# SJLeo/GCC

Measured on AMD Instinct MI355X. Metric: training images/sec at 256x256 (pix2pix GCC), higher is better.
Workload: dtype bf16; 1 GPU; Pix2Pix cityscapes 256x256 GCC distill+darts iteration (optimize_parameters + optimizer_netD_arch), student ngf32 / masked PatchGAN ndf128, teacher ngf64 / ndf128, filter_cfgs=None (no pretrained checkpoint to prune); batch_per_gpu=16, global_batch=16, image=256x256, parallelism=dp1, dropout=on (counter RNG; the oracle / golden iterations run --no_dropout)

## Files before the change

### gcc_amd/csrc/conv_wgrad.hip

```cpp
#include <mutex>
#include <string.h>
#include "common.hpp"

namespace {

struct WgradParams {
    const bf16_t* x;
    const bf16_t* dy;
    float* out;
    int N, H, W, ldx, xoff, Cip, Ci;
    int Ho, Wo, ldy, yoff, Co;
    int KH, KW, stride, pad;
    int ncols;
    int M;
    int ksteps_per_split;
    int col_tiles, co_tiles;
    uint32_t x_bytes, dy_bytes;
    FastDiv dHW, dW, dCip, dKW;
    int batch;
    long x_bstride, dy_bstride;
    int direct;
    int accumulate;
    float* dw;
    int rowmode;
    int debug;
};

constexpr int TP = 64;
constexpr uint32_t OOB = 0x7FFFFFF0u;

template <bool BIG>
struct WCfg {
    static constexpr int WAVES = BIG ? 8 : 4;
    static constexpr int NT = WAVES * 64;
    static constexpr int TCOL = BIG ? 256 : 128;
    static constexpr int TCO = BIG ? 256 : 128;
    static constexpr int RS = TCOL * 2;
    static constexpr int TILE_BYTES = TP * RS;
    static constexpr int CPR = RS / 16;
    static constexpr int RPP = 64 / CPR;
    static constexpr int WCOL = BIG ? 128 : 64;
    static constexpr int FI = WCOL / 16;
    static constexpr int FJ = 4;
    static constexpr int CH = BIG ? 16 : 8;
    static constexpr int TBL_BYTES = 2 * CH * TP * 8;
    static constexpr int LDS_BYTES = 4 * TILE_BYTES + TBL_BYTES;
};

__device__ __forceinline__ int phys_col_bytes(int row, int col_bytes) {
    return ((((col_bytes >> 5) ^ (row & 7)) << 5) | (col_bytes & 31));
}

template <int RS>
__device__ __forceinline__ bf16x8 tr_frag(const char* tile, int ks, int colbase, int lane) {
    const int g = lane >> 4, i = lane & 15;
    const int r0 = ks * 32 + 4 * g + (i >> 2), r1 = r0 + 16;
    const int cb = (colbase + 4 * (i & 3)) * 2;
    s16x4 lo = __builtin_amdgcn_ds_read_tr16_b64_v4i16(LDS_PTR(s16x4, tile + r0 * RS + phys_col_bytes(r0, cb)));
    s16x4 hi = __builtin_amdgcn_ds_read_tr16_b64_v4i16(LDS_PTR(s16x4, tile + r1 * RS + phys_col_bytes(r1, cb)));
    s16x8 v = {lo[0], lo[1], lo[2], lo[3], hi[0], hi[1], hi[2], hi[3]};
    return __builtin_bit_cast(bf16x8, v);
}

template <bool BIG, bool TABLE>
__device__ __forceinline__ void wgrad_body(const WgradParams& p, const int tile, const int split, const int bidx, char* smem) {
    using C = WCfg<BIG>;
    constexpr int RS = C::RS, TILE_BYTES = C::TILE_BYTES, FI = C::FI, FJ = C::FJ;
    char* sX = smem;
    char* sY = smem + 2 * TILE_BYTES;

    const int tid = threadIdx.x, lane = tid & 63;
    const int wave = __builtin_amdgcn_readfirstlane(tid >> 6);
    const int wa = wave & 1, wb = wave >> 1;

    const int ct = tile % p.col_tiles;
    const int ot = tile / p.col_tiles;
    const int col0 = ct * C::TCOL, co0 = ot * C::TCO;
    const int k_begin = split * p.ksteps_per_split;
    int k_end = k_begin + p.ksteps_per_split;
    const int ksteps_total = (p.M + TP - 1) / TP;
    if (k_end > ksteps_total) k_end = ksteps_total;

    const i32x4 rs_x = make_rsrc(p.x + (size_t)bidx * p.x_bstride, p.x_bytes);
    const i32x4 rs_y = make_rsrc(p.dy + (size_t)bidx * p.dy_bstride, p.dy_bytes);
    const uint32_t lds0 = (uint32_t)(uintptr_t)LDS_PTR(char, smem);

    const int rsub = lane / C::CPR, pch = lane % C::CPR;
    int q_tap_dy[4], q_tap_dx[4], q_cx[4], q_coy[4];
    bool q_colok[4], q_cook[4];
    int cxl[4], cyl[4];
    uint32_t xbits[4];
#pragma unroll
    for (int i = 0; i < 4; i++) {
        const int r7 = (C::RPP * (4 * wave + i) + rsub) & 7;
        const int lch = (((pch >> 1) ^ r7) << 1) | (pch & 1);
        const int q = col0 + lch * 8;
        q_colok[i] = q < p.ncols;
        const int tap = fdiv(q, p.dCip);
        q_cx[i] = q - tap * p.Cip;
        const int kh = fdiv(tap, p.dKW);
        const int kw = tap - kh * p.KW;
        q_tap_dy[i] = kh - p.pad; q_tap_dx[i] = kw - p.pad;
        q_coy[i] = co0 + lch * 8;
        q_cook[i] = q_coy[i] < ((p.Co + 7) & ~7);
        cxl[i] = ((kh * p.W + kw) * p.ldx + q_cx[i]) * 2;
        cyl[i] = q_cook[i] ? ((C::RPP * (4 * wave + i) + rsub) * p.ldy + p.yoff + q_coy[i]) * 2 : (int)0x80000000u;
        xbits[i] = q_colok[i] ? (0x80000000u | (1u << (kh & 15)) | (1u << (16 + (kw & 15)))) : 0x80008000u;
    }

    char* tbl = smem + 4 * TILE_BYTES;
    const int nk = k_end - k_begin;
    auto build_chunk = [&](int c) {
        for (int e = tid; e < C::CH * TP; e += C::NT) {
            const int step = c * C::CH + (e >> 6);
            const int m = (k_begin + step) * TP + (e & 63);
            i32x2 ent = {0, 0};
            if (step < nk && m < p.M) {
                const int n = fdiv(m, p.dHW);
                const int r = m - n * (p.Ho * p.Wo);
                const int oy = fdiv(r, p.dW);
                const int ox = r - oy * p.Wo;
                const int iy0 = oy * p.stride - p.pad, ix0 = ox * p.stride - p.pad;
                uint32_t mask = 0x80000000u;
                for (int k = 0; k < p.KH; k++) mask |= ((unsigned)(iy0 + k) < (unsigned)p.H) ? (1u << k) : 0u;
                for (int k = 0; k < p.KW; k++) mask |= ((unsigned)(ix0 + k) < (unsigned)p.W) ? (1u << (16 + k)) : 0u;
                ent[0] = (((n * p.H + iy0) * p.W + ix0) * p.ldx + p.xoff) * 2;
                ent[1] = (int)mask;
            }
            *(i32x2*)(tbl + ((c & 1) * (C::CH * TP) + e) * 8) = ent;
        }
    };
    const int tl = (C::RPP * 4 * wave + rsub) * 8;
    auto issue_loads = [&](int kstep, int stage) {
        const char* te = tbl + (kstep & (2 * C::CH - 1)) * (TP * 8) + tl;
        const int sby = (k_begin + kstep) * TP * p.ldy * 2;
#pragma unroll
        for (int i = 0; i < 4; i++) {
            uint32_t offx, offy;
            if constexpr (!TABLE) {
                const int row = C::RPP * (4 * wave + i) + rsub;
                const int m = (k_begin + kstep) * TP + row;
                const bool mv = m < p.M;
                const int n = fdiv(m, p.dHW);
                const int r = m - n * (p.Ho * p.Wo);
                const int oy = fdiv(r, p.dW);
                const int ox = r - oy * p.Wo;
                const int iy = oy * p.stride + q_tap_dy[i], ix = ox * p.stride + q_tap_dx[i];
                const bool okx = mv && q_colok[i] && (unsigned)iy < (unsigned)p.H && (unsigned)ix < (unsigned)p.W;
                offx = okx ? (uint32_t)((((n * p.H + iy) * p.W + ix) * p.ldx + p.xoff + q_cx[i]) * 2) : OOB;
                const bool oky = mv && q_cook[i];
                offy = oky ? (uint32_t)((m * p.ldy + p.yoff + q_coy[i]) * 2) : OOB;
            } else {
                const i32x2 ent = *(const i32x2*)(te + i * (C::RPP * 8));
                const uint32_t mask = (uint32_t)ent[1];
// ... 269 lines not shown
    const int split = blockIdx.z;
    const int b_begin = split * p.blocks_per_split;
    int b_end = b_begin + p.blocks_per_split;
    if (b_end > p.blocks) b_end = p.blocks;
    const int nb = b_end - b_begin;

    const i32x4 rs_x = make_rsrc(p.x, p.x_bytes);
    const i32x4 rs_y = make_rsrc(p.dy, p.dy_bytes);
    const uint32_t lds0 = (uint32_t)(uintptr_t)LDS_PTR(char, smem);

    const int rsub = lane >> 3, pch = lane & 7;
    int yl[YJ], ypy[YJ], ypx[YJ];
#pragma unroll
    for (int j = 0; j < YJ; j++) {
        const int row = 8 * (wave + NW * j) + rsub;
        const int lch = (((pch >> 1) ^ ((row >> 1) & 3)) << 1) | (pch & 1);
        ypy[j] = row >> 4; ypx[j] = row & 15;
        yl[j] = ((ypy[j] * p.Wo + ypx[j]) * p.ldy + p.yoff + co0 + lch * 8) * 2;
    }
    int xl[XJ], xhy[XJ], xhx[XJ];
#pragma unroll
    for (int j = 0; j < XJ; j++) {
        const int row = 8 * (wave + NW * j) + rsub;
        const int lch = (((pch >> 1) ^ ((row >> 1) & 3)) << 1) | (pch & 1);
        xhy[j] = row / HP; xhx[j] = row - xhy[j] * HP;
        xl[j] = ((xhy[j] * p.W + xhx[j]) * p.ldx + p.xoff + ci0 + lch * 8) * 2;
        if (xhx[j] >= HW) xhx[j] = 1 << 20;
    }
    const int mine = ((C::YP - 1 - wave) / NW + 1) + ((C::XP - 1 - wave) / NW + 1);
    auto issue = [&](int b, int stage) {
        const int n = fdiv(b, p.dT);
        const int t = b - n * (p.TY * p.TX);
        const int ty = fdiv(t, p.dTX);
        const int Y0 = ty * TR, X0 = (t - ty * p.TX) * TW;
        const int ybase = ((n * p.Ho + Y0) * p.Wo + X0) * p.ldy * 2;
        const int xbase = ((n * p.H + Y0 - 1) * p.W + X0 - 1) * p.ldx * 2;
        const uint32_t d0 = lds0 + stage * STAGE;
#pragma unroll
        for (int j = 0; j < YJ; j++) {
            if ((j + 1) * NW <= C::YP || wave + NW * j < C::YP) {
                const bool ok = Y0 + ypy[j] < p.Ho && X0 + ypx[j] < p.Wo;
                lds_dma16(rs_y, d0 + (wave + NW * j) * 1024, ok ? (uint32_t)(ybase + yl[j]) : OOB);
            }
        }
#pragma unroll
        for (int j = 0; j < XJ; j++) {
            if ((j + 1) * NW <= C::XP || wave + NW * j < C::XP) {
                const bool ok = (unsigned)(Y0 - 1 + xhy[j]) < (unsigned)p.H && (unsigned)(X0 - 1 + xhx[j]) < (unsigned)p.W;
                lds_dma16(rs_x, d0 + Y_BYTES + (wave + NW * j) * 1024, ok ? (uint32_t)(xbase + xl[j]) : OOB);
            }
        }
    };

    const int g = lane >> 4, li = lane & 15;
    const int px = 4 * g + (li >> 2);
    const int kh = KS == 4 ? wave >> 1 : wave / 3, kw0 = KS == 4 ? 2 * (wave & 1) : wave - 3 * (wave / 3);
    int ya[4], xa[TPW][4];
#pragma unroll
    for (int t = 0; t < 4; t++) {
        ya[t] = px * RSB + ((t ^ ((px >> 1) & 3)) << 5) + 8 * (li & 3);
#pragma unroll
        for (int tj = 0; tj < TPW; tj++) {
            const int hrow = kh * HP + px + kw0 + tj;
            xa[tj][t] = Y_BYTES + hrow * RSB + ((t ^ ((hrow >> 1) & 3)) << 5) + 8 * (li & 3);
        }
    }

    f32x4 acc[TPW][4][4];
#pragma unroll
    for (int a = 0; a < TPW; a++)
#pragma unroll
        for (int i = 0; i < 4; i++)
#pragma unroll
            for (int j = 0; j < 4; j++) acc[a][i][j] = f32x4{0.f, 0.f, 0.f, 0.f};

    if (nb > 0) {
        issue(b_begin, 0);
        if (nb > 1) issue(b_begin + 1, 1);
        int cur = 0, fill = 2;
        for (int b = 0; b < nb; b++) {
            if (b + 1 < nb) {
                if (mine == 7) asm volatile("s_waitcnt vmcnt(7)" ::: "memory");
                else if (mine == 6) asm volatile("s_waitcnt vmcnt(6)" ::: "memory");
                else if (mine == 5) asm volatile("s_waitcnt vmcnt(5)" ::: "memory");
                else asm volatile("s_waitcnt vmcnt(4)" ::: "memory");
            } else {
                asm volatile("s_waitcnt vmcnt(0)" ::: "memory");
            }
            __syncthreads();
            if (b + 2 < nb) issue(b_begin + b + 2, fill);
            const char* st = smem + cur * STAGE;
#pragma unroll
            for (int pp = 0; pp < 2; pp++) {
                bf16x8 fx[2][TPW * 4], fy[2][4];
#pragma unroll
                for (int k2 = 0; k2 < 2; k2++) {
                    const int ks = 2 * pp + k2;
#pragma unroll
                    for (int tj = 0; tj < TPW; tj++)
#pragma unroll
                        for (int t = 0; t < 4; t++)
                            fx[k2][tj * 4 + t] = ts_frag(st + xa[tj][t] + 2 * ks * (HP * RSB), HP * RSB);
#pragma unroll
                    for (int t = 0; t < 4; t++) fy[k2][t] = ts_frag(st + ya[t] + 2 * ks * (TW * RSB), TW * RSB);
                }
#pragma unroll
                for (int k2 = 0; k2 < 2; k2++)
#pragma unroll
                    for (int i = 0; i < TPW * 4; i++)
#pragma unroll
                        for (int j = 0; j < 4; j++)
                            acc[i >> 2][i & 3][j] = __builtin_amdgcn_mfma_f32_16x16x32_bf16(fx[k2][i], fy[k2][j], acc[i >> 2][i & 3][j], 0, 0, 0);
                if constexpr (KS == 4) {
                    __builtin_amdgcn_sched_group_barrier(0x100, 24, 0);
#pragma unroll
                    for (int r = 0; r < 12; r++) {
                        __builtin_amdgcn_sched_group_barrier(0x008, 2, 0);
                        __builtin_amdgcn_sched_group_barrier(0x100, 2, 0);
                    }
                    __builtin_amdgcn_sched_group_barrier(0x008, 40, 0);
                } else {
                    __builtin_amdgcn_sched_group_barrier(0x100, 16, 0);
#pragma unroll
                    for (int r = 0; r < 8; r++) {
                        __builtin_amdgcn_sched_group_barrier(0x008, 2, 0);
                        __builtin_amdgcn_sched_group_barrier(0x100, 2, 0);
                    }
                    __builtin_amdgcn_sched_group_barrier(0x008, 16, 0);
                }
            }
            cur = cur == NS - 1 ? 0 : cur + 1;
            fill = fill == NS - 1 ? 0 : fill + 1;
        }
    }

    float* slab = p.direct ? p.dw : p.out + (size_t)split * p.Co * p.ncols;
    const bool rmw = p.direct && p.accumulate;
#pragma unroll
    for (int j = 0; j < 4; j++) {
        const int co = co0 + j * 16 + (lane & 15);
#pragma unroll
        for (int tj = 0; tj < TPW; tj++)
#pragma unroll
            for (int i = 0; i < 4; i++) {
                const int col = (TPW * wave + tj) * p.Ci + ci0 + i * 16 + 4 * (lane >> 4);
                f32x4* d = (f32x4*)(slab + (size_t)co * p.ncols + col);
                f32x4 v = acc[tj][i][j];
                if (rmw) { const f32x4 o = *d; v[0] += o[0]; v[1] += o[1]; v[2] += o[2]; v[3] += o[3]; }
                *d = v;
            }
    }
}

int ts_plan(const gcc_conv_t* c, int batch, int* blocks_per_split) {
    const int mode = gcc_opt(GCC_OPT_WGRAD_TS);
    const bool k4 = c->KH == 4 && c->KW == 4, k3 = c->KH == 3 && c->KW == 3;
    if (!mode || batch != 1 || !(k4 || k3) || c->stride != 1 || c->pad != 1) return 0;
    if ((c->Ci & 63) || (c->Co & 63) || c->H < 2 || c->W < 2) return 0;
    const int Ho = k4 ? c->H - 1 : c->H, Wo = k4 ? c->W - 1 : c->W;
    const int blocks = c->N * cdiv(Ho, ts::TR) * cdiv(Wo, ts::TW);
    const int tiles = (c->Ci / 64) * (c->Co / 64);
    const int target = plan_or(c->plan.wgrad_wgs_big, PLAN_WGRAD_WGS_BIG);
    int splits = tiles >= (target * 25) / 32 ? 1 : cdiv(target, tiles);
    if (mode == 1) {
        if (k4) {
            const int max_splits = blocks / 16;
            if (max_splits < 1 || tiles < 32) return 0;
            if (splits > max_splits) splits = max_splits;
        } else {
            const int max_splits = blocks / 8;
            if (splits > max_splits) splits = max_splits;
            if (splits < 1 || (long)tiles * splits < 128) return 0;
        }
    } else if (splits > blocks) {
        splits = blocks;
    }
    const int per = cdiv(blocks, splits);
    *blocks_per_split = per;
    return cdiv(blocks, per);
}

int plan_splits(const gcc_conv_t* c, int batch, int* ksteps_per_split, bool* big_out = nullptr) {
    const int Ho = gcc_conv_out(c->H, c->KH, c->stride, c->pad), Wo = gcc_conv_out(c->W, c->KW, c->stride, c->pad);
    const long M = (long)c->N * Ho * Wo;
    const int ksteps = (int)((M + TP - 1) / TP);
    const int ncols = c->KH * c->KW * ceil8(c->Ci);
    constexpr int BIG_MIN_TILES = 8;
    const int tiles_big = cdiv(ncols, 256) * cdiv(c->Co, 256);
    bool big = batch == 1 && (c->Ci & 7) == 0 && c->Co >= 256 && ncols >= 256 && tiles_big >= BIG_MIN_TILES && ksteps >= 64;
    int splits;
    if (big) {
        const int target = plan_or(c->plan.wgrad_wgs_big, PLAN_WGRAD_WGS_BIG);
        splits = tiles_big >= (target * 25) / 32 ? 1 : cdiv(target, tiles_big);
        const int max_splits = ksteps / 16 > 0 ? ksteps / 16 : 1;
        if (splits > max_splits) splits = max_splits;
    } else {
        const int tiles = cdiv(ncols, 128) * cdiv(c->Co, 128) * batch;
        const int target = plan_or(c->plan.wgrad_wgs, PLAN_WGRAD_WGS);
        splits = tiles >= (target * 3) / 8 ? 1 : cdiv(target, tiles);
        const int max_splits = ksteps / 8 > 0 ? ksteps / 8 : 1;
        if (splits > max_splits) splits = max_splits;
    }
    if (splits < 1) splits = 1;
    const int per = cdiv(ksteps, splits);
    splits = cdiv(ksteps, per);
    *ksteps_per_split = per;
    if (big_out) *big_out = big;
    return splits;
}

}

size_t gcc_internal_wgrad_workspace(const gcc_conv_t* c, int batch) {
    if (!c || c->Ci <= 0 || c->Co <= 0 || batch < 1) return 0;
    int per, tper;
    int splits = plan_splits(c, batch, &per);
    const int tsplits = ts_plan(c, batch, &tper);
    if (tsplits > splits) splits = tsplits;
    return (size_t)splits * batch * c->Co * c->KH * c->KW * ceil8(c->Ci) * sizeof(float);
}

size_t gcc_internal_head_gather_bytes(const gcc_conv_t* c);
int gcc_internal_head_gather(const gcc_conv_t* c, const void* dy, void* g, hipStream_t st);
static size_t al256(size_t v) { return (v + 255) & ~(size_t)255; }
static gcc_conv_t head_conv1x1(const gcc_conv_t* c) {
    const int taps = c->KH * c->KW;
    gcc_conv_t c1 = {c->N, c->H, c->W, c->Ci, taps * 8, 1, 1, 1, 0, c->ldx, c->xoff, taps * 8, 0};
    return c1;
}
static size_t head_wgrad_workspace(const gcc_conv_t* c) {
    const size_t g = gcc_internal_head_gather_bytes(c);
    if (!g) return 0;
    const gcc_conv_t c1 = head_conv1x1(c);
    return al256(g) + al256((size_t)c1.Co * ceil8(c->Ci) * sizeof(float)) + gcc_internal_wgrad_workspace(&c1, 1);
}
__global__ void head_rows_fold_kernel(const float* __restrict__ big, float* __restrict__ dw, int taps, int Cip, int accumulate) {
    const int n = taps * Cip;
    for (int i = blockIdx.x * blockDim.x + threadIdx.x; i < n; i += gridDim.x * blockDim.x) {
        const int t = i / Cip, cc = i - t * Cip;
        const float v = big[(size_t)(t * 8) * Cip + cc];
        dw[i] = accumulate ? dw[i] + v : v;
    }
}

size_t gcc_internal_thinout_wgrad_workspace(const gcc_conv_t* c);
int gcc_internal_thinout_wgrad(const gcc_conv_t* c, const void* x, const void* dy, float* dw, int accumulate, void* ws, size_t ws_bytes,
                               hipStream_t st);

extern "C" size_t gcc_conv_wgrad_workspace(const gcc_conv_t* c) {
    const size_t h = c ? head_wgrad_workspace(c) : 0;
    if (h) return h;
    const size_t t = c ? gcc_internal_thinout_wgrad_workspace(c) : 0, g = gcc_internal_wgrad_workspace(c, 1);
    return t > g ? t : g;
}

int gcc_internal_wgrad(const gcc_conv_t* c, const void* x, const void* dy, float* dw, int accumulate, void* ws,
                       size_t ws_bytes, int batch, long x_bstride, long dy_bstride, hipStream_t st, int rows_l,
                       int cols_l, int row_split, int col_split) {
    GCC_ENTER();
    if (!c || !x || !dy || !dw || !ws) return GCC_ERR_BAD_ARG;
    if (c->N <= 0 || c->H <= 0 || c->W <= 0 || c->Ci <= 0 || c->Co <= 0 || c->KH <= 0 || c->KW <= 0 ||
        c->stride <= 0 || c->pad < 0)
        return GCC_ERR_BAD_ARG;
    if ((c->ldx & 7) || (c->xoff & 7) || (c->ldy & 7) || (c->yoff & 7)) return GCC_ERR_BAD_ARG;
    const int Ho = gcc_conv_out(c->H, c->KH, c->stride, c->pad), Wo = gcc_conv_out(c->W, c->KW, c->stride, c->pad);
    if (Ho <= 0 || Wo <= 0) return GCC_ERR_BAD_ARG;
    if (batch < 1 || ws_bytes < gcc_internal_wgrad_workspace(c, batch)) return GCC_ERR_WORKSPACE;
    WgradParams p;
    p.x = (const bf16_t*)x; p.dy = (const bf16_t*)dy; p.out = (float*)ws;
    p.N = c->N; p.H = c->H; p.W = c->W; p.ldx = c->ldx; p.xoff = c->xoff; p.Ci = c->Ci; p.Cip = ceil8(c->Ci);
    p.Ho = Ho; p.Wo = Wo; p.ldy = c->ldy; p.yoff = c->yoff; p.Co = c->Co;
    p.KH = c->KH; p.KW = c->KW; p.stride = c->stride; p.pad = c->pad;
    p.ncols = c->KH * c->KW * p.Cip;
    const size_t M = (size_t)c->N * Ho * Wo;
    const size_t xb = (size_t)c->N * c->H * c->W * c->ldx * 2, yb = M * c->ldy * 2;
    if (xb >= OOB || yb >= OOB || M >= (1u << 30)) return GCC_ERR_UNSUPPORTED;
    p.M = (int)M; p.x_bytes = (uint32_t)xb; p.dy_bytes = (uint32_t)yb;
    bool big = false;
    const int splits = plan_splits(c, batch, &p.ksteps_per_split, &big);
    p.batch = batch; p.x_bstride = x_bstride; p.dy_bstride = dy_bstride;
    const bool seg = rows_l > 0;
    const bool regular = !seg && (c->Ci & 7) == 0 && (((uintptr_t)dw) & 15) == 0;
    big = big && regular;
    p.direct = (splits == 1 && regular) ? 1 : 0;
    p.accumulate = accumulate; p.dw = dw;
    p.debug = gcc_diag_bits();
    p.rowmode = (c->KH <= 15 && c->KW <= 15) ? 1 : 0;
    int tper = 0;
    const int tsplits = regular ? ts_plan(c, batch, &tper) : 0;
    if (tsplits > 0) {
        TsParams t;
        t.x = p.x; t.dy = p.dy; t.out = (float*)ws; t.dw = dw;
        t.N = c->N; t.H = c->H; t.W = c->W; t.ldx = c->ldx; t.xoff = c->xoff; t.Ci = c->Ci;
        t.Ho = Ho; t.Wo = Wo; t.ldy = c->ldy; t.yoff = c->yoff; t.Co = c->Co;
        t.ncols = p.ncols;
        t.ci_tiles = c->Ci / 64; t.co_tiles = c->Co / 64;
        t.TY = cdiv(Ho, ts::TR); t.TX = cdiv(Wo, ts::TW);
        t.blocks = c->N * t.TY * t.TX; t.blocks_per_split = tper;
        t.x_bytes = p.x_bytes; t.dy_bytes = p.dy_bytes;
        t.dT = make_fastdiv(t.TY * t.TX); t.dTX = make_fastdiv(t.TX);
        t.direct = tsplits == 1 ? 1 : 0; t.accumulate = accumulate;
        static std::once_flag ts_once;
        static bool ts_attr_ok = false;
        std::call_once(ts_once, [] {
            ts_attr_ok = hipFuncSetAttribute((const void*)wgrad_ts_kernel<4>, hipFuncAttributeMaxDynamicSharedMemorySize, TsCfg<4>::LDS_BYTES) == hipSuccess &&
                         hipFuncSetAttribute((const void*)wgrad_ts_kernel<3>, hipFuncAttributeMaxDynamicSharedMemorySize, TsCfg<3>::LDS_BYTES) == hipSuccess;
        });
        if (!ts_attr_ok) return GCC_ERR_LAUNCH;
        if (c->KH == 4)
            hipLaunchKernelGGL(wgrad_ts_kernel<4>, dim3(t.ci_tiles * t.co_tiles, 1, tsplits), dim3(TsCfg<4>::NT), TsCfg<4>::LDS_BYTES, st, t);
        else
            hipLaunchKernelGGL(wgrad_ts_kernel<3>, dim3(t.ci_tiles * t.co_tiles, 1, tsplits), dim3(TsCfg<3>::NT), TsCfg<3>::LDS_BYTES, st, t);
        GCC_CHECK_LAUNCH();
        if (t.direct) return GCC_OK;
        const size_t n4 = (size_t)c->Co * p.ncols / 4;
        if (tsplits <= 8) {
            int blocks = (int)((n4 + 255) / 256);
            if (blocks > 8192) blocks = 8192;
            hipLaunchKernelGGL(wgrad_reduce_flat_kernel, dim3(blocks), dim3(256), 0, st, (const float*)ws, dw, tsplits, n4, accumulate);
        } else {
            int blocks = (int)((n4 + 63) / 64);
            if (blocks > 4096) blocks = 4096;
            hipLaunchKernelGGL(wgrad_reduce_vec_kernel, dim3(blocks), dim3(256), 0, st, (const float*)ws, dw, tsplits, n4, accumulate);
        }
        GCC_CHECK_LAUNCH();
        return GCC_OK;
    }
    const int tcol = big ? 256 : 128;
    p.col_tiles = cdiv(p.ncols, tcol); p.co_tiles = cdiv(c->Co, tcol);
    p.dHW = make_fastdiv(Ho * Wo); p.dW = make_fastdiv(Wo); p.dCip = make_fastdiv(p.Cip); p.dKW = make_fastdiv(c->KW);
    static std::once_flag attr_once;
    std::call_once(attr_once, [] {
        hipFuncSetAttribute((const void*)wgrad_kernel<false, false>, hipFuncAttributeMaxDynamicSharedMemorySize, WCfg<false>::LDS_BYTES);
        hipFuncSetAttribute((const void*)wgrad_kernel<true, false>, hipFuncAttributeMaxDynamicSharedMemorySize, WCfg<true>::LDS_BYTES);
        hipFuncSetAttribute((const void*)wgrad_kernel<false, true>, hipFuncAttributeMaxDynamicSharedMemorySize, WCfg<false>::LDS_BYTES);
        hipFuncSetAttribute((const void*)wgrad_kernel<true, true>, hipFuncAttributeMaxDynamicSharedMemorySize, WCfg<true>::LDS_BYTES);
    });
    const dim3 grid(p.col_tiles * p.co_tiles, batch, splits);
    if (big && p.rowmode)
        hipLaunchKernelGGL((wgrad_kernel<true, true>), grid, dim3(WCfg<true>::NT), WCfg<true>::LDS_BYTES, st, p);
    else if (big)
        hipLaunchKernelGGL((wgrad_kernel<true, false>), grid, dim3(WCfg<true>::NT), WCfg<true>::LDS_BYTES, st, p);
    else if (p.rowmode)
        hipLaunchKernelGGL((wgrad_kernel<false, true>), grid, dim3(WCfg<false>::NT), WCfg<false>::LDS_BYTES, st, p);
    else
        hipLaunchKernelGGL((wgrad_kernel<false, false>), grid, dim3(WCfg<false>::NT), WCfg<false>::LDS_BYTES, st, p);
    GCC_CHECK_LAUNCH();
    if (p.direct) return GCC_OK;
    const size_t total = (size_t)batch * c->Co * c->KH * c->KW * c->Ci;
    if (regular) {
        const size_t n4 = total / 4;
        if (splits <= 8) {
            int blocks = (int)((n4 + 255) / 256);
            if (blocks > 8192) blocks = 8192;
            hipLaunchKernelGGL(wgrad_reduce_flat_kernel, dim3(blocks), dim3(256), 0, st, (const float*)ws, dw, splits, n4,
                               accumulate);
        } else {
            int blocks = (int)((n4 + 63) / 64);
            if (blocks > 4096) blocks = 4096;
            hipLaunchKernelGGL(wgrad_reduce_vec_kernel, dim3(blocks), dim3(256), 0, st, (const float*)ws, dw, splits, n4,
                               accumulate);
        }
    } else {
        const size_t outs = seg ? (size_t)rows_l * c->KH * c->KW * cols_l : total;
        const bool deep = splits >= 32;
        int blocks = (int)((outs + (deep ? 15 : 63)) / (deep ? 16 : 64));
        if (blocks > 4096) blocks = 4096;
        const int rows = seg ? rows_l : batch * c->Co, cols = seg ? cols_l : c->Ci, cop = seg ? c->Co : batch * c->Co;
        const int rsp = seg ? row_split : 0, csp = seg ? col_split : 0;
        if (deep)
            hipLaunchKernelGGL((wgrad_reduce_kernel<16, 16>), dim3(blocks), dim3(256), 0, st, (const float*)ws, dw, splits, rows,
                               c->KH * c->KW, cols, p.Cip, accumulate, cop, rsp, csp);
        else
            hipLaunchKernelGGL((wgrad_reduce_kernel<64, 4>), dim3(blocks), dim3(256), 0, st, (const float*)ws, dw, splits, rows,
                               c->KH * c->KW, cols, p.Cip, accumulate, cop, rsp, csp);
    }
    GCC_CHECK_LAUNCH();
    return GCC_OK;
}

extern "C" int gcc_conv_wgrad(const gcc_conv_t* c, const void* x, const void* dy, float* dw, int accumulate,
                              void* ws, size_t ws_bytes, gcc_stream_t stream) {
    GCC_ENTER();
    const size_t hw = c ? head_wgrad_workspace(c) : 0;
    if (hw && ws && ws_bytes >= hw && x && dy && dw && (c->Ci & 7) == 0) {
        hipStream_t st = (hipStream_t)stream;
        char* base = (char*)ws;
        const gcc_conv_t c1 = head_conv1x1(c);
        const size_t gbytes = al256(gcc_internal_head_gather_bytes(c));
        const size_t bbytes = al256((size_t)c1.Co * c->Ci * sizeof(float));
        int rc = gcc_internal_head_gather(c, dy, base, st);
        if (rc) return rc;
        float* big = (float*)(base + gbytes);
        rc = gcc_internal_wgrad(&c1, x, base, big, 0, base + gbytes + bbytes, ws_bytes - gbytes - bbytes, 1, 0, 0, st, 0, 0, 0, 0);
        if (rc) return rc;
        const int taps = c->KH * c->KW;
        hipLaunchKernelGGL(head_rows_fold_kernel, dim3((taps * c->Ci + 255) / 256), dim3(256), 0, st, (const float*)big, dw, taps, c->Ci,
                           accumulate);
        GCC_CHECK_LAUNCH();
        return GCC_OK;
    }
    if (c && x && dy && dw && ws && (((uintptr_t)dw) & 3) == 0) {
        const int rc = gcc_internal_thinout_wgrad(c, x, dy, dw, accumulate, ws, ws_bytes, (hipStream_t)stream);
        if (rc != GCC_ERR_UNSUPPORTED) return rc;
    }
    return gcc_internal_wgrad(c, x, dy, dw, accumulate, ws, ws_bytes, 1, 0, 0, (hipStream_t)stream, 0, 0, 0, 0);
}

extern "C" int gcc_conv_wgrad_seg(const gcc_conv_t* c, const void* x, const void* dy, float* dw, int rows, int cols,
                                  int row_split, int col_split, int accumulate, void* ws, size_t ws_bytes,
                                  gcc_stream_t stream) {
    GCC_ENTER();
    if (!c || rows <= 0 || cols <= 0) return GCC_ERR_BAD_ARG;
    if (c->Co != seg_phys_size(rows, row_split) || c->Ci != seg_phys_size(cols, col_split)) return GCC_ERR_BAD_ARG;
    return gcc_internal_wgrad(c, x, dy, dw, accumulate, ws, ws_bytes, 1, 0, 0, (hipStream_t)stream, rows, cols, row_split,
                              col_split);
}

namespace {
struct GroupPlan {
    int n, total_wgs;
    int per[GROUP_MAX], splits[GROUP_MAX], tiles[GROUP_MAX], order[GROUP_MAX];
    size_t slab_off[GROUP_MAX], ws_bytes;
};
int group_cus() {
    static const int v = [] {
        int dev = 0, n = 0;
        if (hipGetDevice(&dev) != hipSuccess || hipDeviceGetAttribute(&n, hipDeviceAttributeMultiprocessorCount, dev) != hipSuccess || n <= 0) {
            (void)hipGetLastError();
            n = 256;
        }
        return n;
    }();
    return v;
}
bool group_item_ok(const gcc_wgrad_item_t* it) {
    const gcc_conv_t* c = &it->c;
    if (c->N <= 0 || c->H <= 0 || c->W <= 0 || c->Ci <= 0 || c->Co <= 0 || c->KH <= 0 || c->KW <= 0 || c->stride <= 0 || c->pad < 0) return false;
    if ((c->Ci & 7) || (c->ldx & 7) || (c->xoff & 7) || (c->ldy & 7) || (c->yoff & 7)) return false;
    if (c->KH > 15 || c->KW > 15) return false;
    const int Ho = gcc_conv_out(c->H, c->KH, c->stride, c->pad), Wo = gcc_conv_out(c->W, c->KW, c->stride, c->pad);
    if (Ho <= 0 || Wo <= 0) return false;
    const size_t M = (size_t)c->N * Ho * Wo;
    if ((size_t)c->N * c->H * c->W * c->ldx * 2 >= OOB || M * c->ldy * 2 >= OOB || M >= (1u << 30)) return false;
    if (head_wgrad_workspace(c) || gcc_internal_thinout_wgrad_workspace(c)) return false;
    int tper = 0;
    if (ts_plan(c, 1, &tper) > 0) return false;
    return true;
}
int group_plan(const gcc_wgrad_item_t* items, int n, GroupPlan* g) {
    if (!items || n < 1 || n > GROUP_MAX) return GCC_ERR_BAD_ARG;
    long work = 0;
    int ksteps[GROUP_MAX];
    for (int i = 0; i < n; i++) {
        if (!group_item_ok(&items[i])) return GCC_ERR_UNSUPPORTED;
        const gcc_conv_t* c = &items[i].c;
        const long M = (long)c->N * gcc_conv_out(c->H, c->KH, c->stride, c->pad) * gcc_conv_out(c->W, c->KW, c->stride, c->pad);
        ksteps[i] = (int)((M + TP - 1) / TP);
        g->tiles[i] = cdiv(c->KH * c->KW * c->Ci, 128) * cdiv(c->Co, 128);
        work += (long)g->tiles[i] * ksteps[i];
    }
    long S = cdiv(work, (long)4 * group_cus());
// ... 102 lines not shown
```

Baseline: 1079 images/s.

## Add tile-staged wgrad kernel for stride-2 4x4 convolutions

Adds a new weight-gradient kernel for 4x4 stride-2 pad-1 convolutions. It stages dy tiles and parity-split input rows into LDS via async DMA with double buffering, then computes all 16 kernel taps with MFMA from the staged data, reusing each dy fragment across kernel rows. ts_plan is extended to route eligible stride-2 convs (batch==1, channel multiples of 64, enough tiles) to this path instead of the generic im2col-style wgrad. It adds heuristic gating and a Python index-model script for checking; the risk is new code paths for downsampling layers, which the PatchGAN and the UNet encoder use heavily.

```diff
diff --git a/gcc_amd/csrc/conv_wgrad.hip b/gcc_amd/csrc/conv_wgrad.hip
--- a/gcc_amd/csrc/conv_wgrad.hip
+++ b/gcc_amd/csrc/conv_wgrad.hip
@@ -1,5 +1,6 @@
 #include <mutex>
 #include <string.h>
+#include <type_traits>
 #include "common.hpp"
 
 namespace {
@@ -575,18 +576,189 @@
     }
 }
 
+struct Ts2Cfg {
+    static constexpr int TR = ts::TR, TW = ts::TW, PX = TR * TW;
+    static constexpr int HP = 24, PW = TW + 1, PL = TR + 1;
+    static constexpr int PROWS = PL * HP, UROWS = 2 * PROWS;
+    static constexpr int XP = UROWS / 8, YP = PX / 8;
+    static constexpr int RSB = 128;
+    static constexpr int Y_BYTES = PX * RSB, X_BYTES = UROWS * RSB;
+    static constexpr int LDS_BYTES = 2 * Y_BYTES + 2 * X_BYTES;
+    static constexpr int NW = 8, NT = NW * 64;
+    static constexpr int YJ = YP / NW, XJ = (XP + NW - 1) / NW;
+    static constexpr int FYK = 3;
+};
+
+__global__ __launch_bounds__(Ts2Cfg::NT) void wgrad_ts2_kernel(const TsParams p) {
+    using C = Ts2Cfg;
+    constexpr int TR = C::TR, TW = C::TW, HP = C::HP, RSB = C::RSB, Y_BYTES = C::Y_BYTES, X_BYTES = C::X_BYTES;
+    constexpr int NW = C::NW, YJ = C::YJ, XJ = C::XJ;
+    extern __shared__ __attribute__((aligned(16))) char smem[];
+    const int tid = threadIdx.x, lane = tid & 63;
+    const int wave = __builtin_amdgcn_readfirstlane(tid >> 6);
+    const int ntiles = gridDim.x;
+    const int unit_id = xcd_remap(blockIdx.x + ntiles * blockIdx.z, ntiles * gridDim.z);
+    const int split = unit_id / ntiles, tile = unit_id - split * ntiles;
+    const int ct = tile % p.ci_tiles, ot = tile / p.ci_tiles;
+    const int ci0 = ct * 64, co0 = ot * 64;
+    const int b_begin = split * p.blocks_per_split;
+    int b_end = b_begin + p.blocks_per_split;
+    if (b_end > p.blocks) b_end = p.blocks;
+    const int nb = b_end - b_begin;
+
+    const i32x4 rs_x = make_rsrc(p.x, p.x_bytes);
+    const i32x4 rs_y = make_rsrc(p.dy, p.dy_bytes);
+    const uint32_t lds0 = (uint32_t)(uintptr_t)LDS_PTR(char, smem);
+
+    const int rsub = lane >> 3, pch = lane & 7;
+    int yl[YJ], ypy[YJ], ypx[YJ];
+#pragma unroll
+    for (int j = 0; j < YJ; j++) {
+        const int row = 8 * (wave + NW * j) + rsub;
+        const int lch = (((pch >> 1) ^ ((row >> 1) & 3)) << 1) | (pch & 1);
+        ypy[j] = row >> 4; ypx[j] = row & 15;
+        yl[j] = ((ypy[j] * p.Wo + ypx[j]) * p.ldy + p.yoff + co0 + lch * 8) * 2;
+    }
+    int xl[XJ], xiy[XJ], xix[XJ];
+#pragma unroll
+    for (int j = 0; j < XJ; j++) {
+        const int row = 8 * (wave + NW * j) + rsub;
+        const int lch = (((pch >> 1) ^ ((row >> 1) & 3)) << 1) | (pch & 1);
+        const int cp = row >= C::PROWS ? 1 : 0, rr = row - cp * C::PROWS;
+        const int L = rr / HP, c = rr - L * HP;
+        xiy[j] = 2 * L; xix[j] = 2 * c + cp;
+        xl[j] = ((xiy[j] * p.W + xix[j]) * p.ldx + p.xoff + ci0 + lch * 8) * 2;
+        if (c >= C::PW) xix[j] = 1 << 20;
+    }
+    auto issue = [&](int u) {
+        const int b = b_begin + (u >> 1), rp = u & 1;
+        const int n = fdiv(b, p.dT);
+        const int t = b - n * (p.TY * p.TX);
+        const int ty = fdiv(t, p.dTX);
+        const int Y0 = ty * TR, X0 = (t - ty * p.TX) * TW;
+        if (rp == 0) {
+            const int ybase = ((n * p.Ho + Y0) * p.Wo + X0) * p.ldy * 2;
+            const uint32_t d0 = lds0 + ((u >> 1) & 1) * Y_BYTES;
+#pragma unroll
+            for (int j = 0; j < YJ; j++) {
+                const bool ok = Y0 + ypy[j] < p.Ho && X0 + ypx[j] < p.Wo;
+                lds_dma16(rs_y, d0 + (wave + NW * j) * 1024, ok ? (uint32_t)(ybase + yl[j]) : OOB);
+            }
+        }
+        const int iy0 = 2 * Y0 + rp - 1, ix0 = 2 * X0 - 1;
+        const int xbase = ((n * p.H + iy0) * p.W + ix0) * p.ldx * 2;
+        const uint32_t d0 = lds0 + 2 * Y_BYTES + rp * X_BYTES;
+#pragma unroll
+        for (int j = 0; j < XJ; j++) {
+            if ((j + 1) * NW <= C::XP || wave + NW * j < C::XP) {
+                const bool ok = (unsigned)(iy0 + xiy[j]) < (unsigned)p.H && (unsigned)(ix0 + xix[j]) < (unsigned)p.W;
+                lds_dma16(rs_x, d0 + (wave + NW * j) * 1024, ok ? (uint32_t)(xbase + xl[j]) : OOB);
+            }
+        }
+    };
+
+    const int g = lane >> 4, li = lane & 15;
+    const int px = 4 * g + (li >> 2);
+    const int hrow = (wave & 1) * C::PROWS + (wave >> 2) * HP + px + ((wave >> 1) & 1);
+    int ya[4], xa[4];
+#pragma unroll
+    for (int t = 0; t < 4; t++) {
+        ya[t] = px * RSB + ((t ^ ((px >> 1) & 3)) << 5) + 8 * (li & 3);
+        xa[t] = 2 * Y_BYTES + hrow * RSB + ((t ^ ((hrow >> 1) & 3)) << 5) + 8 * (li & 3);
+    }
+
+    f32x4 acc[2][4][4];
+#pragma unroll
+    for (int a = 0; a < 2; a++)
+#pragma unroll
+        for (int i = 0; i < 4; i++)
+#pragma unroll
+            for (int j = 0; j < 4; j++) acc[a][i][j] = f32x4{0.f, 0.f, 0.f, 0.f};
+
+    auto unit = [&](auto RPc, int b, const char* sy, bf16x8 (&fy)[4][4]) {
+        constexpr int rp = decltype(RPc)::value;
+        constexpr int R[4] = {rp && 3 >= 4 - C::FYK ? 8 : 16, rp && 2 >= 4 - C::FYK ? 8 : 16, rp && 1 >= 4 - C::FYK ? 8 : 16, rp && 0 >= 4 - C::FYK ? 8 : 16};
+        asm volatile("s_waitcnt vmcnt(0)" ::: "memory");
+        __syncthreads();
+        if (rp == 0 || b + 1 < nb) issue(2 * b + rp + 1);
+        const char* sx = smem + rp * X_BYTES;
+        bf16x8 fx[2][4];
+        auto reads = [&](int s) {
+            const int ks = rp ? 3 - s : s;
+#pragma unroll
+            for (int t = 0; t < 4; t++) fx[s & 1][t] = ts_frag(sx + xa[t] + 2 * ks * (HP * RSB), HP * RSB);
+            if (!(rp && ks >= 4 - C::FYK)) {
+#pragma unroll
+                for (int t = 0; t < 4; t++) fy[ks][t] = ts_frag(sy + ya[t] + 2 * ks * (TW * RSB), TW * RSB);
+            }
+        };
+        reads(0);
+#pragma unroll
+        for (int s = 0; s < 4; s++) {
+            if (s < 3) reads(s + 1);
+            const int ks = rp ? 3 - s : s;
+#pragma unroll
+            for (int i = 0; i < 4; i++)
+#pragma unroll
+                for (int j = 0; j < 4; j++)
+                    acc[rp][i][j] = __builtin_amdgcn_mfma_f32_16x16x32_bf16(fx[s & 1][i], fy[ks][j], acc[rp][i][j], 0, 0, 0);
+        }
+        __builtin_amdgcn_sched_group_barrier(0x100, R[0], 0);
+#pragma unroll
+        for (int r = 0; r < R[1] / 2; r++) { __builtin_amdgcn_sched_group_barrier(0x008, 2, 0); __builtin_amdgcn_sched_group_barrier(0x100, 2, 0); }
+        if constexpr (R[1] < 16) __builtin_amdgcn_sched_group_barrier(0x008, 16 - R[1], 0);
+#pragma unroll
+        for (int r = 0; r < R[2] / 2; r++) { __builtin_amdgcn_sched_group_barrier(0x008, 2, 0); __builtin_amdgcn_sched_group_barrier(0x100, 2, 0); }
+        if constexpr (R[2] < 16) __builtin_amdgcn_sched_group_barrier(0x008, 16 - R[2], 0);
+#pragma unroll
+        for (int r = 0; r < R[3] / 2; r++) { __builtin_amdgcn_sched_group_barrier(0x008, 2, 0); __builtin_amdgcn_sched_group_barrier(0x100, 2, 0); }
+        if constexpr (R[3] < 16) __builtin_amdgcn_sched_group_barrier(0x008, 16 - R[3], 0);
+        __builtin_amdgcn_sched_group_barrier(0x008, 16, 0);
+    };
+
+    if (nb > 0) {
+        issue(0);
+        for (int b = 0; b < nb; b++) {
+            const char* sy = smem + (b & 1) * Y_BYTES;
+            bf16x8 fy[4][4];
+            unit(std::integral_constant<int, 0>(), b, sy, fy);
+            unit(std::integral_constant<int, 1>(), b, sy, fy);
+        }
+    }
+
+    float* slab = p.direct ? p.dw : p.out + (size_t)split * p.Co * p.ncols;
+    const bool rmw = p.direct && p.accumulate;
+#pragma unroll
+    for (int j = 0; j < 4; j++) {
+        const int co = co0 + j * 16 + (lane & 15);
+#pragma unroll
+        for (int rp = 0; rp < 2; rp++)
+#pragma unroll
+            for (int i = 0; i < 4; i++) {
+                const int col = (4 * (rp + 2 * (wave >> 2)) + (wave & 3)) * p.Ci + ci0 + i * 16 + 4 * (lane >> 4);
+                f32x4* d = (f32x4*)(slab + (size_t)co * p.ncols + col);
+                f32x4 v = acc[rp][i][j];
+                if (rmw) { const f32x4 o = *d; v[0] += o[0]; v[1] += o[1]; v[2] += o[2]; v[3] += o[3]; }
+                *d = v;
+            }
+    }
+}
+
 int ts_plan(const gcc_conv_t* c, int batch, int* blocks_per_split) {
     const int mode = gcc_opt(GCC_OPT_WGRAD_TS);
     const bool k4 = c->KH == 4 && c->KW == 4, k3 = c->KH == 3 && c->KW == 3;
-    if (!mode || batch != 1 || !(k4 || k3) || c->stride != 1 || c->pad != 1) return 0;
+    const bool s2 = k4 && c->stride == 2;
+    if (!mode || batch != 1 || !(k4 || k3) || !(c->stride == 1 || s2) || c->pad != 1) return 0;
     if ((c->Ci & 63) || (c->Co & 63) || c->H < 2 || c->W < 2) return 0;
-    const int Ho = k4 ? c->H - 1 : c->H, Wo = k4 ? c->W - 1 : c->W;
+    const int Ho = s2 ? c->H / 2 : k4 ? c->H - 1 : c->H, Wo = s2 ? c->W / 2 : k4 ? c->W - 1 : c->W;
     const int blocks = c->N * cdiv(Ho, ts::TR) * cdiv(Wo, ts::TW);
     const int tiles = (c->Ci / 64) * (c->Co / 64);
     const int target = plan_or(c->plan.wgrad_wgs_big, PLAN_WGRAD_WGS_BIG);
     int splits = tiles >= (target * 25) / 32 ? 1 : cdiv(target, tiles);
     if (mode == 1) {
-        if (k4) {
+        if (s2) {
+            if (tiles < 8 || splits > blocks / 16 || (long)tiles * blocks < 4096) return 0;
+        } else if (k4) {
             const int max_splits = blocks / 16;
             if (max_splits < 1 || tiles < 32) return 0;
             if (splits > max_splits) splits = max_splits;
@@ -727,10 +899,13 @@
         static bool ts_attr_ok = false;
         std::call_once(ts_once, [] {
             ts_attr_ok = hipFuncSetAttribute((const void*)wgrad_ts_kernel<4>, hipFuncAttributeMaxDynamicSharedMemorySize, TsCfg<4>::LDS_BYTES) == hipSuccess &&
-                         hipFuncSetAttribute((const void*)wgrad_ts_kernel<3>, hipFuncAttributeMaxDynamicSharedMemorySize, TsCfg<3>::LDS_BYTES) == hipSuccess;
+                         hipFuncSetAttribute((const void*)wgrad_ts_kernel<3>, hipFuncAttributeMaxDynamicSharedMemorySize, TsCfg<3>::LDS_BYTES) == hipSuccess &&
+                         hipFuncSetAttribute((const void*)wgrad_ts2_kernel, hipFuncAttributeMaxDynamicSharedMemorySize, Ts2Cfg::LDS_BYTES) == hipSuccess;
         });
         if (!ts_attr_ok) return GCC_ERR_LAUNCH;
-        if (c->KH == 4)
+        if (c->stride == 2)
+            hipLaunchKernelGGL(wgrad_ts2_kernel, dim3(t.ci_tiles * t.co_tiles, 1, tsplits), dim3(Ts2Cfg::NT), Ts2Cfg::LDS_BYTES, st, t);
+        else if (c->KH == 4)
             hipLaunchKernelGGL(wgrad_ts_kernel<4>, dim3(t.ci_tiles * t.co_tiles, 1, tsplits), dim3(TsCfg<4>::NT), TsCfg<4>::LDS_BYTES, st, t);
         else
             hipLaunchKernelGGL(wgrad_ts_kernel<3>, dim3(t.ci_tiles * t.co_tiles, 1, tsplits), dim3(TsCfg<3>::NT), TsCfg<3>::LDS_BYTES, st, t);
diff --git a/scratch/model_wgrad_ts_s2.py b/scratch/model_wgrad_ts_s2.py
--- /dev/null
+++ b/scratch/model_wgrad_ts_s2.py
@@ -0,0 +1,71 @@
+TR, TW, HP, PW, PL = 8, 16, 24, 17, 9
+PROWS, UROWS = PL * HP, 2 * PL * HP
+NW, XP = 8, UROWS // 8
+
+
+def stage_unit(N, H, W, ldx, xoff, ci0, n, Y0, X0, rp):
+    rows = {}
+    iy0, ix0 = 2 * Y0 + rp - 1, 2 * X0 - 1
+    xbase = ((n * H + iy0) * W + ix0) * ldx
+    for wave in range(NW):
+        for j in range((XP + NW - 1) // NW):
+            piece = wave + NW * j
+            if piece >= XP:
+                continue
+            for lane in range(64):
+                rsub, pch = lane >> 3, lane & 7
+                row = 8 * piece + rsub
+                lch = (((pch >> 1) ^ ((row >> 1) & 3)) << 1) | (pch & 1)
+                cp = 1 if row >= PROWS else 0
+                rr = row - cp * PROWS
+                L, c = rr // HP, rr % HP
+                xiy, xix = 2 * L, 2 * c + cp
+                xl = (xiy * W + xix) * ldx + xoff + ci0 + lch * 8
+                if c >= PW:
+                    xix = 1 << 20
+                ok = 0 <= iy0 + xiy < H and 0 <= ix0 + xix < W
+                off = xbase + xl if ok else None
+                if ok:
+                    assert 0 <= off and off + 8 <= N * H * W * ldx, (off, 'out of the buffer')
+                rows[(row, pch)] = (off, lch)
+    return rows
+
+
+def check(N, H, W, ldx=72, xoff=8, ci0=0):
+    Ho, Wo = H // 2, W // 2
+    assert Ho == (H + 2 - 4) // 2 + 1 and Wo == (W + 2 - 4) // 2 + 1
+    TY, TX = -(-Ho // TR), -(-Wo // TW)
+    checked = 0
+    for n in range(N):
+        for ty in range(TY):
+            for tx in range(TX):
+                Y0, X0 = ty * TR, tx * TW
+                for rp in range(2):
+                    rows = stage_unit(N, H, W, ldx, xoff, ci0, n, Y0, X0, rp)
+                    for wave in range(NW):
+                        kh, kw = rp + 2 * (wave >> 2), wave & 3
+                        for ks in range(4):
+                            for half in range(2):
+                                py = 2 * ks + half
+                                for px in range(TW):
+                                    hrow0 = (wave & 1) * PROWS + (wave >> 2) * HP + px + ((wave >> 1) & 1)
+                                    hrow = hrow0 + (2 * ks + half) * HP
+                                    assert hrow < UROWS
+                                    assert ((hrow >> 1) & 3) == ((hrow0 >> 1) & 3)
+                                    oy, ox = Y0 + py, X0 + px
+                                    iy, ix = 2 * oy + kh - 1, 2 * ox + kw - 1
+                                    for t in range(4):
+                                        for h in range(2):
+                                            pchunk = ((t ^ ((hrow >> 1) & 3)) << 1) | h
+                                            off, lch = rows[(hrow, pchunk)]
+                                            assert lch == 2 * t + h
+                                            if oy < Ho and ox < Wo:
+                                                want = ((n * H + iy) * W + ix) * ldx + xoff + ci0 + lch * 8 if 0 <= iy < H and 0 <= ix < W else None
+                                                assert off == want, (n, Y0, X0, rp, wave, py, px, off, want)
+                                                checked += 1
+    return checked
+
+
+if __name__ == '__main__':
+    for (N, H, W) in [(2, 9, 21), (1, 37, 29), (2, 16, 16), (1, 2, 2), (1, 32, 32), (2, 20, 70), (1, 18, 34), (1, 3, 5)]:
+        print('N %d  %3d x %3d : %d fragment chunks agree with the convolution' % (N, H, W, check(N, H, W)))
```

After: 1084 images/s, median of 6. Within noise of the previous version (+0.5%).
